# jason-gideon/GPUMounter

Hardware: AMD Instinct MI355X
Metric: p50_gpu_attach_latency_ms (lower is better)
Workload: dtype none

## Files before the change

gpumounter_amd/_native.py:

```python
from __future__ import annotations

import ctypes as C
import os
import subprocess
import threading
from typing import Optional

LIB_DIR = os.path.join(os.path.dirname(os.path.abspath(__file__)), "_lib")
NATIVE_DIR = os.path.join(os.path.dirname(os.path.dirname(os.path.abspath(__file__))), "native")

_lock = threading.Lock()
_libs: dict = {}


class NativeError(RuntimeError):
    pass


def lib_path(name: str) -> str:
    return os.path.join(LIB_DIR, name)


def build(target: str = "all", quiet: bool = True) -> None:
    import fcntl
# ... 71 lines not shown
def mock_smi() -> C.CDLL:
    lib = _load("libamd_smi_mock.so", "host")
    lib.gm_mock_set_procs_file.argtypes = [C.c_char_p]
    lib.gm_mock_set_ecc.argtypes = [C.c_uint32, C.c_uint64, C.c_uint64]
    return lib


class DevRule(C.Structure):
    _fields_ = [("type", C.c_char), ("access", C.c_uint8), ("allow", C.c_uint8),
                ("pad", C.c_uint8), ("major", C.c_int32), ("minor", C.c_int32)]


class DevNode(C.Structure):
    _fields_ = [("path", C.c_char * 112), ("major", C.c_uint32), ("minor", C.c_uint32),
                ("mode", C.c_uint32), ("uid", C.c_int32), ("gid", C.c_int32)]


class BpfTiming(C.Structure):
    _fields_ = [("query_ns", C.c_uint64), ("map_ns", C.c_uint64), ("build_ns", C.c_uint64),
                ("load_ns", C.c_uint64), ("attach_ns", C.c_uint64), ("programs", C.c_uint32),
                ("insns", C.c_uint32)]


HOST_ABI_VERSION = 6
GM_ACC_MKNOD, GM_ACC_READ, GM_ACC_WRITE = 1, 2, 4
GM_DEV_EMULATE, GM_DEV_VIA_SETNS, GM_DEV_REPLACE, GM_DEV_BIND = 1, 2, 4, 8


def host() -> C.CDLL:
    lib = _load("libgm_host.so", "host")
    if not getattr(lib, "_gm_typed", False):
        abi = lib.gm_host_abi_version()
        if abi != HOST_ABI_VERSION:
            raise RuntimeError(f"libgm_host.so ABI {abi} != {HOST_ABI_VERSION} expected: stale "
                               f"build, run `make -C native`")
        lib.gm_cg1_apply.argtypes = [C.c_char_p, C.POINTER(DevRule), C.c_int]
        lib.gm_cg1_format_rule.argtypes = [C.POINTER(DevRule), C.c_char_p, C.c_int]
        lib.gm_bpf_dev_build.argtypes = [C.POINTER(DevRule), C.c_int, C.c_int, C.c_int,
                                         C.POINTER(C.c_uint64), C.c_int]
        lib.gm_bpf_dev_load.argtypes = [C.POINTER(C.c_uint64), C.c_int, C.c_char_p, C.c_char_p,
                                        C.c_int]
        lib.gm_bpf_dev_query.argtypes = [C.c_char_p, C.POINTER(C.c_uint32), C.c_uint32,
                                         C.POINTER(C.c_uint32), C.POINTER(C.c_uint32)]
        lib.gm_bpf_prog_name.argtypes = [C.c_uint32, C.c_char_p, C.c_int]
        lib.gm_bpf_dev_program.argtypes = [C.c_char_p, C.POINTER(C.c_uint64), C.c_uint32,
                                           C.POINTER(C.c_uint32), C.POINTER(C.c_uint32)]
        lib.gm_bpf_dev_program_at.argtypes = [C.c_char_p, C.c_uint32, C.c_int,
# ... 5 lines not shown
                                           C.POINTER(C.c_uint32), C.POINTER(C.c_uint32)]
        lib.gm_bpf_dev_restore.argtypes = [C.c_char_p, C.c_char_p]
        lib.gm_bpf_dev_build_set.argtypes = [C.c_int, C.POINTER(DevRule), C.c_int, C.c_int,
                                             C.c_int, C.POINTER(C.c_uint64), C.c_int]
        lib.gm_bpf_dev_probe_set.argtypes = []
        lib.gm_devnodes_bind_probe.argtypes = []
        lib.gm_bpf_dev_straight_line.argtypes = [C.c_int]
        lib.gm_bpf_dev_straight_line.restype = None
        lib.gm_bpf_dev_set_at.argtypes = [C.c_char_p, C.c_uint32, C.POINTER(C.c_uint32),
                                          C.c_uint32, C.POINTER(C.c_uint32),
                                          C.POINTER(C.c_uint32)]
        lib.gm_bpf_dev_last_timing.argtypes = [C.POINTER(BpfTiming)]
        lib.gm_bpf_dev_last_timing.restype = None
        lib.gm_devnodes_create.argtypes = [C.c_int, C.c_char_p, C.POINTER(DevNode), C.c_int,
                                           C.c_int, C.POINTER(C.c_int)]
        lib.gm_devnodes_remove.argtypes = lib.gm_devnodes_create.argtypes
        lib.gm_devnodes_guard.argtypes = [C.c_char_p]
        lib.gm_devnodes_stage.argtypes = [C.c_char_p, C.c_int]
        lib.gm_devnode_stat.argtypes = [C.c_int, C.c_char_p, C.c_char_p, C.c_int,
                                        C.POINTER(C.c_int), C.POINTER(C.c_uint32),
                                        C.POINTER(C.c_uint32), C.POINTER(C.c_uint32)]
        lib.gm_devnodes_present.argtypes = [C.c_int, C.c_char_p, C.POINTER(DevNode), C.c_int,
                                            C.c_int, C.POINTER(C.c_uint8)]
        lib.gm_proc_dev_users.argtypes = [C.c_uint32, C.c_uint32, C.POINTER(C.c_int32), C.c_int,
                                          C.POINTER(C.c_int)]
        lib.gm_proc_scan_devs.argtypes = [C.POINTER(C.c_int32), C.c_int, C.POINTER(C.c_uint32),
                                          C.c_int, C.POINTER(C.c_uint8), C.POINTER(C.c_int32)]
        lib.gm_proc_filter_dev_users.argtypes = [C.POINTER(C.c_int32), C.c_int, C.c_uint32,
                                                 C.c_uint32, C.POINTER(C.c_int32)]
        lib.gm_proc_read_pids.argtypes = [C.c_char_p, C.POINTER(C.c_int32), C.c_int,
                                          C.POINTER(C.c_int)]
        lib.gm_sd_get_device_allow.argtypes = [C.c_char_p, C.c_char_p, C.c_char_p, C.c_int,
                                               C.c_char_p, C.c_int]
        lib.gm_sd_set_device_allow.argtypes = [C.c_char_p, C.c_char_p, C.POINTER(C.c_char_p),
                                               C.POINTER(C.c_char_p), C.c_int, C.c_int,
                                               C.c_char_p, C.c_int]
        lib.gm_sd_unit_path.argtypes = [C.c_char_p, C.c_char_p, C.c_int]
        lib.gm_roctx_push.argtypes = [C.c_char_p]
        lib.gm_roctx_mark.argtypes = [C.c_char_p]
        lib.gm_roctx_start.argtypes = [C.c_char_p]
        lib.gm_roctx_start.restype = C.c_uint64
        lib.gm_roctx_stop.argtypes = [C.c_uint64]
        lib.gm_roctx_stop.restype = None
        lib.gm_now_ns.restype = C.c_uint64
        lib._gm_typed = True
    return lib
# ... 125 lines not shown
```

gpumounter_amd/node/cgroup.py:

```python
from __future__ import annotations

import ctypes as C
import errno
import functools
import glob
import json
import os
from abc import ABC, abstractmethod
from typing import Dict, FrozenSet, Iterable, List, Optional, Sequence, Set, Tuple

from gpumounter_amd import _native
from gpumounter_amd.models.device import DeviceNode
from gpumounter_amd.models.pod import (QOS_BESTEFFORT, QOS_BURSTABLE, ContainerRef, qos_class,
                                       uid_of)
from gpumounter_amd.node import bpfvm
from gpumounter_amd.utils import log, trace

_log = log.get("node.cgroup")

RUNTIME_SCOPE_PREFIXES = ("cri-containerd-", "docker-", "crio-", "containerd-", "")
FAKE_MARKER = ".gm_fake"
BPF_STATE = "gm.bpf.json"


class CgroupError(RuntimeError):
    pass


def _esc(s: str) -> str:
    return s.replace("-", "_")


class CgroupResolver:
    def __init__(self, root: str = "/sys/fs/cgroup", mode: str = "auto", driver: str = "auto",
                 proc_root: str = "/proc"):
        self.root = root
        self.proc_root = proc_root
        self.mode = self.detect_mode(root) if mode == "auto" else mode
        self.base = os.path.join(root, "devices") if self.mode == "v1" else root
        self.driver = driver
        self._cache: Dict[Tuple[str, str], str] = {}

    @staticmethod
    def detect_mode(root: str) -> str:
        if os.path.isdir(os.path.join(root, "devices")):
            return "v1"
        if os.path.exists(os.path.join(root, "cgroup.controllers")):
            return "v2"
        return "v2"
# ... 60 lines not shown
                with open(os.path.join(self.proc_root, pid, "cgroup")) as fh:
                    lines = fh.read().splitlines()
            except OSError:
                continue
            for line in lines:
                parts = line.split(":", 2)
                if len(parts) != 3 or container_id not in parts[2]:
                    continue
                ctrls = parts[1].split(",") if parts[1] else [""]
                if want_ctrl not in ctrls:
                    continue
                cand = os.path.join(self.base, parts[2].lstrip("/"))
                if os.path.isdir(cand):
                    return cand
        return None

    def forget(self, pod_uid: str) -> None:
        for k in [k for k in self._cache if k[0] == pod_uid]:
            del self._cache[k]

    @staticmethod
    def pids(cgdir: str, recursive: bool = True) -> List[int]:
        lib = _native.host()
        out: List[int] = []
        buf = (C.c_int32 * 4096)()
        n = C.c_int(0)
        stack = [cgdir]
        while stack:
            d = stack.pop()
            path = os.path.join(d, "cgroup.procs")
            rc = lib.gm_proc_read_pids(path.encode(), buf, 4096, C.byref(n))
            if rc < 0 and rc != -errno.ENOENT:
                raise CgroupError(f"read {path}: {os.strerror(-rc)}")
            if rc >= 0:
                out.extend(buf[:min(n.value, 4096)])
            if recursive:
                try:
                    with os.scandir(d) as it:
                        stack.extend(e.path for e in it if e.is_dir(follow_symlinks=False))
                except (FileNotFoundError, NotADirectoryError):
                    pass
        return sorted(set(out))


def rules_for(nodes: Iterable[DeviceNode], allow: bool, access: str = "rw") -> List[_native.DevRule]:
    acc = 0
    if "r" in access:
        acc |= _native.GM_ACC_READ
    if "w" in access:
        acc |= _native.GM_ACC_WRITE
    if "m" in access:
        acc |= _native.GM_ACC_MKNOD
    return [_native.DevRule(b"c", acc, 1 if allow else 0, 0, n.major, n.minor) for n in nodes]


def _rule_array(rules: Sequence[_native.DevRule]):
    arr = (_native.DevRule * max(len(rules), 1))()
    for i, r in enumerate(rules):
        arr[i] = r
    return arr


def format_rule(r: _native.DevRule) -> str:
    buf = C.create_string_buffer(64)
    _native.host().gm_cg1_format_rule(C.byref(r), buf, 64)
# ... 434 lines not shown
```

gpumounter_amd/node/devnodes.py:

```python
from __future__ import annotations

import ctypes as C
import errno
import os
from dataclasses import dataclass
from typing import List, Optional, Sequence, Tuple

from gpumounter_amd import _native
from gpumounter_amd.models.device import DeviceNode
from gpumounter_amd.utils import log


class DevNodeError(RuntimeError):
    def __init__(self, msg: str, results: Sequence[int] = ()):
        super().__init__(msg)
        self.results = list(results)


@dataclass(frozen=True)
class Target:

    pid: int = 0
    root: str = ""


CREATED, PRESENT, SHARED_HOST = 0, 1, 2

_log = log.get("node.devnodes")


class DevNodeWriter:

    def __init__(self, mode: str = "procroot", host_dev: str = "", userns: str = "auto",
                 stage_dir: str = "", proc_root: str = "/proc") -> None:
        self.mode = mode
        self.userns = userns
        self.stage_dir = stage_dir
        self.proc_root = proc_root
        self._staged = False
        self._own_userns = self._userns_id("self")
        self.flags = 0
        if mode == "setns":
            self.flags |= _native.GM_DEV_VIA_SETNS
        if mode == "emulate":
            self.flags |= _native.GM_DEV_EMULATE
        self.host_dev = host_dev
        rc = _native.host().gm_devnodes_guard(host_dev.encode() if host_dev else None)
        if rc < 0:
            _log.warning("host /dev guard off: cannot read %s (%s)", host_dev, os.strerror(-rc))
        self.guarded = max(rc, 0)

    @staticmethod
    def _array(nodes: Sequence[DeviceNode], owner: Tuple[int, int] = (-1, -1)):
        arr = (_native.DevNode * max(len(nodes), 1))()
        for i, n in enumerate(nodes):
            rel = n.path.lstrip("/").encode()
            if len(rel) >= 112:
                raise DevNodeError(f"path too long: {n.path}")
            arr[i].path = rel
            arr[i].major = n.major
            arr[i].minor = n.minor
            arr[i].mode = n.mode
            arr[i].uid, arr[i].gid = owner
        return arr

    def _mntns(self, pid) -> Optional[str]:
        try:
            return os.readlink(f"{self.proc_root}/{pid}/ns/mnt")
        except OSError:
            return None

    def root_pid(self, pids: Sequence[int]) -> int:
        if self.mode == "emulate":
            return pids[0] if pids else 0
        own = self._mntns("self")
        for pid in pids:
            ns = self._mntns(pid)
            if ns is not None and ns != own:
                return pid
        return 0

    def _userns_id(self, pid) -> Optional[Tuple[int, int]]:
        try:
            st = os.stat(f"{self.proc_root}/{pid}/ns/user")
        except OSError:
            return None
        return st.st_dev, st.st_ino

    def _bind(self, t: Target) -> bool:
        if self.userns == "bind":
            return True
        if self.userns != "auto" or self.mode == "emulate" or t.root or t.pid <= 0:
            return False
        theirs = self._userns_id(t.pid)
        return theirs is not None and self._own_userns is not None and theirs != self._own_userns

    def _mapped_root(self, t: Target) -> Tuple[int, int]:
        if t.pid <= 0:
            return -1, -1
        out = []
        for f in ("uid_map", "gid_map"):
            host = -1
            try:
# ... 17 lines not shown
        try:
            os.makedirs(os.path.dirname(self.stage_dir.rstrip("/")) or "/", exist_ok=True)
        except OSError as e:
            raise DevNodeError(f"staging directory {self.stage_dir}: {e.strerror}") from e
        rc = _native.host().gm_devnodes_stage(self.stage_dir.encode(), 1)
        if rc < 0:
            raise DevNodeError(f"staging tmpfs at {self.stage_dir}: {os.strerror(-rc)}")
        self._staged = True

    def _call(self, t: Target):
        if not self._bind(t):
            return self.flags, (-1, -1)
        self._ensure_stage()
        return self.flags | _native.GM_DEV_BIND, self._mapped_root(t)

    def _target_args(self, t: Target) -> Tuple[int, Optional[bytes]]:
        if t.root:
            return 0, t.root.encode()
        if t.pid <= 0:
            raise DevNodeError("container has no process to resolve its root from "
                               "(empty cgroup.procs)")
        return t.pid, None

    def create(self, t: Target, nodes: Sequence[DeviceNode]) -> List[int]:
        if not nodes:
            return []
        pid, root = self._target_args(t)
        flags, owner = self._call(t)
        res = (C.c_int * len(nodes))()
        fails = _native.host().gm_devnodes_create(pid, root, self._array(nodes, owner),
                                                  len(nodes), flags, res)
        results = [int(res[i]) for i in range(len(nodes))]
        if fails:
            bad = [(n.path, os.strerror(-r)) for n, r in zip(nodes, results) if r < 0]
            what = "bind mount" if flags & _native.GM_DEV_BIND else "mknod"
            raise DevNodeError(f"{what} failed: {bad}", results)
        return results

    def remove(self, t: Target, nodes: Sequence[DeviceNode]) -> List[int]:
        if not nodes:
            return []
        pid, root = self._target_args(t)
        flags, _ = self._call(t)
        res = (C.c_int * len(nodes))()
        fails = _native.host().gm_devnodes_remove(pid, root, self._array(nodes), len(nodes),
                                                  flags, res)
        results = [int(res[i]) for i in range(len(nodes))]
        if fails and not flags & _native.GM_DEV_BIND and \
                any(r == -errno.EBUSY for r in results) and self.mode != "emulate":
            busy = [i for i, r in enumerate(results) if r == -errno.EBUSY]
            self._ensure_stage()
            sub = [nodes[i] for i in busy]
            res2 = (C.c_int * len(sub))()
            _native.host().gm_devnodes_remove(pid, root, self._array(sub), len(sub),
                                              flags | _native.GM_DEV_BIND, res2)
            for k, i in enumerate(busy):
                results[i] = int(res2[k])
            fails = sum(1 for r in results if r < 0)
        if fails:
            if all(r in (-errno.ESRCH, -errno.ENOENT) for r in results if r < 0):
# ... 37 lines not shown
```

gpumounter_amd/node/hotmount.py:

```python
from __future__ import annotations

import os
from dataclasses import dataclass, field
from typing import Dict, List, Optional, Sequence

from gpumounter_amd.hw.inventory import Inventory
from gpumounter_amd.models.device import AmdGpu, DeviceNode, kfd_node
from gpumounter_amd.models.pod import ContainerRef, running_containers
from gpumounter_amd.node.cgroup import CgroupError, CgroupResolver, DeviceRuleBackend
from gpumounter_amd.node.devnodes import CREATED, DevNodeError, DevNodeWriter, Target
from gpumounter_amd.node.journal import InjectionJournal
from gpumounter_amd.utils import log, trace

_log = log.get("node.hotmount")


class MountError(RuntimeError):
    pass


@dataclass
class ContainerTarget:
    ref: ContainerRef
    cgdir: str
    target: Target
    pids: List[int] = field(default_factory=list)


@dataclass
class AuditIssue:
    container: str
    kind: str
    path: str
    major: int
    minor: int


class HotMount:
    def __init__(self, cfg, inv: Inventory, resolver: CgroupResolver, backend: DeviceRuleBackend,
                 writer: DevNodeWriter, faults=None,
                 journal: Optional[InjectionJournal] = None) -> None:
        from gpumounter_amd.utils.faults import NONE

        self.cfg = cfg
        self.inv = inv
        self.resolver = resolver
        self.backend = backend
        self.writer = writer
        self.faults = faults if faults is not None else NONE
        self.journal = journal if journal is not None else InjectionJournal()
        self.expected: Dict[str, object] = {}

    def _apply(self, cgdir: str, grant, revoke, desired) -> None:
        try:
            self.backend.apply(cgdir, grant, revoke, desired)
        finally:
            fp = getattr(self.backend, "fingerprint", None)
            self.expected[cgdir] = fp(cgdir) if fp is not None else None

    def kfd(self) -> DeviceNode:
        return kfd_node(self.inv.kfd_major)

    def gpu_nodes(self, gpus: Sequence[AmdGpu]) -> List[DeviceNode]:
        out: List[DeviceNode] = []
        for g in sorted(gpus, key=lambda g: g.index):
            out.extend(g.device_nodes(self.cfg.drm_major, self.cfg.inject_card_nodes,
                                      self.cfg.device_file_mode))
        return out

    def managed_nodes(self, hot: Sequence[AmdGpu], base: Sequence[AmdGpu]) -> List[DeviceNode]:
        base_keys = {(n.major, n.minor) for n in self.gpu_nodes(base)}
        nodes = [n for n in self.gpu_nodes(hot) if (n.major, n.minor) not in base_keys]
        if hot and not base:
            nodes.insert(0, self.kfd())
        return nodes

    def targets(self, pod: dict, container: str = "",
                include_privileged: bool = False) -> List[ContainerTarget]:
        refs = [r for r in running_containers(pod, container) if r.running]
        if not refs:
            raise MountError(f"pod {pod['metadata'].get('name')} has no running container"
                             + (f" named {container}" if container else ""))
        out = []
        for r in refs:
            if r.privileged and not include_privileged:
                continue
            cgdir = self.resolver.container_dir(pod, r)
            pids = self.resolver.pids(cgdir)
            if self.cfg.container_root_prefix:
                t = Target(root=os.path.join(self.cfg.container_root_prefix, r.id))
            else:
                t = Target(pid=self.writer.root_pid(pids))
            out.append(ContainerTarget(r, cgdir, t, pids))
        return out

    def _owner(self, pod: dict, t: ContainerTarget) -> dict:
        md = pod.get("metadata", {})
# ... 2 lines not shown

    def resolve(self, pod: dict, container: str = "",
                include_privileged: bool = False) -> List[ContainerTarget]:
        try:
            return self.targets(pod, container, include_privileged)
        except (CgroupError, OSError) as e:
            raise MountError(f"cannot resolve the pod's containers: {e}") from e

    def attach(self, pod: dict, new: Sequence[AmdGpu], have: Sequence[AmdGpu],
               base: Sequence[AmdGpu] = (), container: str = "") -> List[ContainerTarget]:
        before = self.managed_nodes(have, base)
        after = self.managed_nodes(list(have) + list(new), base)
        before_keys = {(n.major, n.minor) for n in before}
        grant = [n for n in after if (n.major, n.minor) not in before_keys]
        with trace.span("resolve"):
            targets = self.resolve(pod, container)
        done: List[tuple] = []
        j = self.journal
        try:
            for t in targets:
                cid = t.ref.id
                known = j.nodes_of(cid)
                with trace.span("devnodes_probe", nodes=len(after)):
                    states = self.writer.present_states(t.target, after)
                theirs = {(n.major, n.minor) for n, st in zip(after, states)
                          if st and (n.major, n.minor) not in known}
                j.intend(cid, [((n.major, n.minor), n.path) for n in grant],
                         [((n.major, n.minor), n.path) for n in after
                          if (n.major, n.minor) not in theirs], **self._owner(pod, t))
                done.append((t, grant, []))
                with trace.span("cgroup_rule", backend=self.backend.name, rules=len(grant)):
                    self.faults.check("cgroup_rule")
                    self._apply(t.cgdir, grant, [], after)
                self.faults.check("cgroup_rule", "after")
                with trace.span("devnodes", nodes=len(after)):
                    self.faults.check("devnodes")
                    res = self.writer.create(t.target, after)
                done[-1] = (t, grant, [n for n, r in zip(after, res) if r == CREATED])
                j.settle(cid, [(n.major, n.minor) for n, r in zip(after, res)
                               if r != CREATED and (n.major, n.minor) not in known
                               and (n.major, n.minor) not in theirs])
                self.faults.check("devnodes", "after")
        except Exception as e:
            self._rollback_attach(done, before)
            for t in targets[len(done):]:
                self._forget_new(t.ref.id, grant, after, before)
            raise MountError(f"attach failed, rolled back: {e}") from e
        return targets

    def _forget_new(self, cid: str, granted, after, before) -> None:
        keep = {(n.major, n.minor) for n in before}
        self.journal.forget(cid, [(n.major, n.minor) for n in granted],
                            [(n.major, n.minor) for n in after if (n.major, n.minor) not in keep])

    def _rollback_attach(self, done, before: List[DeviceNode]) -> None:
        before_keys = {(n.major, n.minor) for n in before}
        for t, granted, created in reversed(done):
            try:
                self.writer.remove(t.target, created)
            except Exception as e:
                _log.error("rollback unlink in %s failed: %s", t.ref.name, e)
            else:
                self.journal.forget(t.ref.id, (), [(n.major, n.minor) for n in created
                                                   if (n.major, n.minor) not in before_keys])
            try:
                try:
                    have = self.backend.installed(t.cgdir)
                    revoke = [n for n in granted if (n.major, n.minor) in have]
                except Exception:
                    revoke = list(granted)
                if revoke:
# ... 105 lines not shown
        if rules:
            self._apply(t.cgdir, [], rules, [])
            self.journal.forget(container_id, [(n.major, n.minor) for n in rules])
        if nodes:
            self.writer.remove(t.target, nodes)
            self.journal.forget(container_id, (), [(n.major, n.minor) for n in nodes])
        return out

    def verify(self, pod: dict, hot: Sequence[AmdGpu], base: Sequence[AmdGpu] = (),
               container: str = "",
               targets: Optional[List[ContainerTarget]] = None) -> List[AuditIssue]:
        want = self.managed_nodes(hot, base)
        issues: List[AuditIssue] = []
        try:
            return self._verify(want, targets if targets is not None
                                else self.targets(pod, container), issues)
        except (CgroupError, DevNodeError, OSError) as e:
            raise MountError(f"read-back failed: {e}") from e

    def _verify(self, want: List[DeviceNode], targets: List[ContainerTarget],
                issues: List[AuditIssue]) -> List[AuditIssue]:
        for t in targets:
            allowed = self.backend.allowed(t.cgdir)
            present = self.writer.present_many(t.target, want)
            for n, ok in zip(want, present):
                if (n.major, n.minor) not in allowed:
                    issues.append(AuditIssue(t.ref.name, "missing_rule", n.path, n.major, n.minor))
                if not ok:
                    issues.append(AuditIssue(t.ref.name, "missing_node", n.path, n.major, n.minor))
        return issues

    def audit(self, pod: dict, hot: Sequence[AmdGpu], base: Sequence[AmdGpu] = (),
              container: str = "") -> List[AuditIssue]:
        want = self.managed_nodes(hot, base)
        want_keys = {(n.major, n.minor) for n in want}
        issues: List[AuditIssue] = []
        base_keys = {(n.major, n.minor) for n in self.gpu_nodes(base)}
        for t in self.targets(pod, container):
            allowed = self.backend.allowed(t.cgdir)
            for n, ok in zip(want, self.writer.present_many(t.target, want)):
                if (n.major, n.minor) not in allowed:
                    issues.append(AuditIssue(t.ref.name, "missing_rule", n.path, n.major, n.minor))
                if not ok:
                    issues.append(AuditIssue(t.ref.name, "missing_node", n.path, n.major, n.minor))
            ent = self.journal.get(t.ref.id)
            if ent is None:
                continue
# ... 21 lines not shown
```

gpumounter_amd/node/journal.py:

```python
from __future__ import annotations

import json
import os
import threading
import time
from dataclasses import dataclass, field
from typing import Dict, Iterable, List, Optional, Tuple

from gpumounter_amd.utils import log

_log = log.get("node.journal")

Key = Tuple[int, int]


@dataclass
class Entry:
    container_id: str
    namespace: str = ""
    pod: str = ""
    pod_uid: str = ""
    container: str = ""
    cgdir: str = ""
    rules: Dict[Key, str] = field(default_factory=dict)
    nodes: Dict[Key, str] = field(default_factory=dict)
    updated: float = 0.0

    def empty(self) -> bool:
        return not self.rules and not self.nodes

    def to_json(self) -> dict:
        return {"container_id": self.container_id, "namespace": self.namespace, "pod": self.pod,
                "pod_uid": self.pod_uid, "container": self.container, "cgdir": self.cgdir,
                "rules": sorted([ma, mi, p] for (ma, mi), p in self.rules.items()),
                "nodes": sorted([ma, mi, p] for (ma, mi), p in self.nodes.items()),
                "updated": self.updated}

    @classmethod
    def from_json(cls, d: dict) -> "Entry":
        return cls(d["container_id"], d.get("namespace", ""), d.get("pod", ""),
                   d.get("pod_uid", ""), d.get("container", ""), d.get("cgdir", ""),
                   {(int(a), int(b)): p for a, b, p in d.get("rules", [])},
                   {(int(a), int(b)): p for a, b, p in d.get("nodes", [])},
                   float(d.get("updated", 0.0)))


def _safe_id(cid: str) -> bool:
    return bool(cid) and all(c.isalnum() or c in "-_." for c in cid) and cid[0] != "."


class InjectionJournal:
    def __init__(self, state_dir: str = "") -> None:
        self.dir = state_dir
        self._entries: Dict[str, Entry] = {}
        self._mu = threading.Lock()
        self.writes = 0
        if state_dir:
            os.makedirs(state_dir, mode=0o700, exist_ok=True)
            self._load()

    def _path(self, cid: str) -> str:
        return os.path.join(self.dir, cid + ".json")

    def _load(self) -> None:
        for fn in os.listdir(self.dir):
            if not fn.endswith(".json"):
                continue
            try:
                with open(os.path.join(self.dir, fn), encoding="utf-8") as fh:
                    e = Entry.from_json(json.load(fh))
# ... 108 lines not shown
```

gpumounter_amd/worker/service.py:

```python
from __future__ import annotations

import asyncio
import contextlib
import json
import secrets
import time
import weakref
from dataclasses import dataclass, field
from typing import Dict, List, Optional, Sequence, Tuple

import grpc

from gpumounter_amd.api import gpu_mount as api
from gpumounter_amd.cluster.correction import Correction, ReserveGate, placement_worse
from gpumounter_amd.cluster.informer import PodInformer
from gpumounter_amd.cluster.kube import ApiError, KubeClient, NotFound
from gpumounter_amd.cluster.placeholder import (InsufficientGPU, Placeholder, PlaceholderManager,
                                                ReserveError)
from gpumounter_amd.cluster.quota import GpuQuota, QuotaExceeded
from gpumounter_amd.hw import topology
from gpumounter_amd.hw.inventory import Inventory
from gpumounter_amd.models import pod as podu
from gpumounter_amd.models.device import AmdGpu, normalize_device_id
from gpumounter_amd.models.types import (ANN_ATTACH_ID, ANN_IDEMPOTENCY, ANN_MOUNT_MODE,
# ... 434 lines not shown
                _log.info("quota refused %d GPU(s) for %s/%s: %s", n, req.namespace,
                          req.pod_name, e)
                self.notify.event(pod, "GPUAttachFailed", str(e), warning=True)
                raise RpcError(grpc.StatusCode.RESOURCE_EXHAUSTED, f"{ERR_QUOTA}: {e}") from e
            except InsufficientGPU as e:
                _log.info("insufficient GPUs on %s: %s", self.cfg.node_name, e)
                self.notify.event(pod, "GPUAttachFailed",
                                  f"{n} GPU(s) requested, node {self.cfg.node_name} cannot "
                                  f"provide them: {e}", warning=True)
                return api.AddGPUResponse(add_gpu_result=api.ADD_INSUFFICIENT, message=str(e))
            except (ReserveError, asyncio.TimeoutError, InjectedFault, LedgerError) as e:
                self._follow_up(pod)
                raise RpcError(grpc.StatusCode.INTERNAL, f"{ERR_INTERNAL}: {e}") from e
            keys = self.inv.by_key()
            new = [keys[normalize_device_id(d)] for d in res.device_ids]
            owner = {}
            for ph in res.placeholders:
                for d in ph.device_ids:
                    owner[keys[normalize_device_id(d)].index] = ph.name
            want = res.preferred or preferred
            if want and sorted(normalize_device_id(d) for d in res.device_ids) != \
                    sorted(normalize_device_id(d) for d in want):
                self.metrics.placement_mismatch.inc()
            try:
                pod = self._current(pod)
                with trace.span("mount", gpus=len(new)):
                    targets = self.hm.attach(pod, new, st.hot, st.own, req.container)
                if self.cfg.attach_verify:
                    with trace.span("verify"):
                        self.faults.check("verify")
                        issues = self.hm.verify(pod, list(st.hot) + new, st.own,
                                                req.container, targets)
                    if issues:
                        self.metrics.verify_failures.inc()
                        raise MountError("attach did not take effect: " + ", ".join(
                            f"{i.container}:{i.kind}:{i.path}" for i in issues[:4]))
            except (MountError, InjectedFault) as e:
                _log.error("mount failed on %s/%s: %s", req.namespace, req.pod_name, e)
                await self._release_or_follow_up(pod, res.placeholders, "a failed mount")
                if await self._rollback(pod, "attach"):
                    return api.AddGPUResponse(add_gpu_result=api.ADD_POD_NOT_FOUND,
                                              message=f"pod went away during the attach: {e}")
                raise RpcError(grpc.StatusCode.INTERNAL, f"{ERR_INTERNAL}: {e}") from e
            if self._owner_gone(pod):
                _log.warning("pod %s/%s was deleted during the attach; releasing its GPUs",
                             req.namespace, req.pod_name)
                await self._release_or_follow_up(pod, res.placeholders, "an attach into a "
                                                                         "deleted pod")
                return api.AddGPUResponse(add_gpu_result=api.ADD_POD_NOT_FOUND,
                                          message="pod went away during the attach")
            msg = "Add GPU Success"
            if lease_exp:
                lease_exp = await self._lease_booked(pod, res.placeholders, lease_exp,
                                                     req.lease_s)
                msg += time.strftime(" (lease until %Y-%m-%dT%H:%M:%SZ)", time.gmtime(lease_exp))
            log.kv(_log, 20, "attached", pod=f"{req.namespace}/{req.pod_name}",
                   gpus=[g.bdf for g in new], by=req.requested_by, lease_s=req.lease_s)
            self.notify.attached(pod, new, list(st.hot) + new,
                                 "entire" if req.is_entire_mount else "single",
# ... 414 lines not shown
```

native/include/gm_host.h:

```cpp
#pragma once
#include <stdint.h>

#ifdef __cplusplus
extern "C" {
#endif

#define GM_HOST_ABI_VERSION 6

#define GM_ACC_MKNOD 1
#define GM_ACC_READ 2
#define GM_ACC_WRITE 4

typedef struct gm_dev_rule {
  char type;
  uint8_t access;
  uint8_t allow;
  uint8_t pad;
  int32_t major;
  int32_t minor;
} gm_dev_rule_t;

int gm_cg1_apply(const char* cgdir, const gm_dev_rule_t* rules, int n);
int gm_cg1_format_rule(const gm_dev_rule_t* rule, char* out, int cap);

int gm_bpf_dev_build(const gm_dev_rule_t* rules, int n, int default_allow, int chain_map_fd,
                     uint64_t* out, int cap);
int gm_bpf_dev_build_set(int set_map_fd, const gm_dev_rule_t* base, int nbase, int default_allow,
                         int chain_map_fd, uint64_t* out, int cap);
int gm_bpf_dev_load(const uint64_t* insns, int n, const char* name, char* log, int logcap);
int gm_bpf_dev_query(const char* cgroup_path, uint32_t* ids, uint32_t cap, uint32_t* n,
// ... 24 lines not shown
  uint32_t minor;
  uint32_t mode;
  int32_t uid;
  int32_t gid;
} gm_dev_node_t;

#define GM_DEV_EMULATE 1
#define GM_DEV_VIA_SETNS 2
#define GM_DEV_REPLACE 4
#define GM_DEV_BIND 8

int gm_devnodes_guard(const char* host_dev);
int gm_devnodes_stage(const char* dir, int mount_tmpfs);
int gm_devnodes_bind_probe(void);
int gm_devnodes_create(int pid, const char* root, const gm_dev_node_t* nodes, int n, int flags,
                       int* results);
int gm_devnodes_remove(int pid, const char* root, const gm_dev_node_t* nodes, int n, int flags,
                       int* results);
int gm_devnode_stat(int pid, const char* root, const char* path, int flags, int* kind,
                    uint32_t* major, uint32_t* minor, uint32_t* mode);
int gm_devnodes_present(int pid, const char* root, const gm_dev_node_t* nodes, int n, int flags,
                        uint8_t* present);

int gm_proc_dev_users(uint32_t major, uint32_t minor, int32_t* pids, int cap, int* n);
int gm_proc_scan_devs(const int32_t* pids, int n, const uint32_t* majmin, int ndev,
                      uint8_t* hits, int32_t* unreadable);
int gm_proc_filter_dev_users(const int32_t* pids, int n, uint32_t major, uint32_t minor,
                             int32_t* out);
int gm_proc_read_pids(const char* path, int32_t* pids, int cap, int* n);

int gm_sd_get_device_allow(const char* bus_path, const char* unit, char* out, int cap, char* err,
                           int errcap);
int gm_sd_set_device_allow(const char* bus_path, const char* unit, const char* const* paths,
                           const char* const* perms, int n, int reset, char* err, int errcap);
int gm_sd_unit_path(const char* unit, char* out, int cap);

int gm_roctx_available(void);
void gm_roctx_push(const char* name);
void gm_roctx_pop(void);
void gm_roctx_mark(const char* name);
uint64_t gm_roctx_start(const char* name);
void gm_roctx_stop(uint64_t id);
uint64_t gm_now_ns(void);

int gm_host_abi_version(void);

#ifdef __cplusplus
}
#endif
```

native/src/gm_host.cpp:

```cpp
#include "gm_host.h"

#include <dirent.h>
#include <dlfcn.h>
#include <errno.h>
#include <fcntl.h>
#include <linux/bpf.h>
#include <sched.h>
#include <signal.h>
#include <stdio.h>
#include <stdlib.h>
#include <string.h>
#include <sys/mount.h>
#include <sys/stat.h>
#include <sys/syscall.h>
#include <sys/sysmacros.h>
#include <time.h>
#include <unistd.h>

#include <atomic>
#include <map>
#include <mutex>
#include <string>
#include <thread>
#include <vector>

namespace {

constexpr const char* kProgName = "gm_devallow";

struct Fd {
  int fd = -1;
  Fd() = default;
  explicit Fd(int f) : fd(f) {}
  Fd(const Fd&) = delete;
  Fd& operator=(const Fd&) = delete;
  Fd(Fd&& o) noexcept : fd(o.fd) { o.fd = -1; }
  Fd& operator=(Fd&& o) noexcept {
    if (this != &o) {
      reset();
      fd = o.fd;
      o.fd = -1;
// ... 797 lines not shown
  std::string leaf;
  int e = w.parent(n.path, false, &pfd, &leaf);
  if (e == -ENOENT) return 1;
  if (e != 0) return e;
  if (guarded_dir(pfd)) return kSharedHost;
  int kind;
  uint32_t maj, min, mode;
  e = stat_leaf(pfd, leaf, &kind, &maj, &min, &mode);
  if (e < 0) return e;
  if (kind == 0) return 1;
  int mounted = is_mount_leaf(pfd, leaf);
  if (mounted < 0) return mounted;
  if (!mounted) {
    if (kind == 3 && is_placeholder(pfd, leaf)) {
      if (unlinkat(pfd, leaf.c_str(), 0) < 0) return -errno;
      return 0;
    }
    return remove_one(w, n);
  }
  if (!(kind == 1 && maj == n.major && min == n.minor)) return -EEXIST;
  if ((e = unmount_leaf(pfd, leaf)) < 0) return e;
  if (is_placeholder(pfd, leaf) && unlinkat(pfd, leaf.c_str(), 0) < 0) return -errno;
  return 0;
}

struct Roctx {
  std::once_flag once;
  int (*push)(const char*) = nullptr;
  int (*pop)() = nullptr;
  void (*mark)(const char*) = nullptr;
  uint64_t (*start)(const char*) = nullptr;
  void (*stop)(uint64_t) = nullptr;
};
Roctx g_roctx;

void roctx_init() {
  std::call_once(g_roctx.once, []() {
    const char* env = getenv("GM_ROCTX");
    if (env && strcmp(env, "0") == 0) return;
    const char* libs[] = {"librocprofiler-sdk-roctx.so.1", "librocprofiler-sdk-roctx.so",
                          "/opt/rocm/lib/librocprofiler-sdk-roctx.so.1"};
    void* dl = nullptr;
    for (const char* l : libs) {
      dl = dlopen(l, RTLD_NOW | RTLD_GLOBAL);
      if (dl) break;
    }
// ... 497 lines not shown
  }
  int fd = open(dir, O_PATH | O_DIRECTORY | O_NOFOLLOW | O_CLOEXEC);
  if (fd < 0) return -errno;
  g_stage_fd = fd;
  return 0;
}

int gm_devnodes_create(int pid, const char* root, const gm_dev_node_t* nodes, int n, int flags,
                       int* results) {
  int failures = 0;
  std::vector<Fd> trees;
  if (flags & GM_DEV_BIND) {
    for (int i = 0; i < n; ++i) {
      int t = staged_tree(nodes[i]);
      if (t < 0) {
        for (int j = 0; j < n; ++j) results[j] = t;
        return n;
      }
      trees.emplace_back(t);
    }
  }
  int e = with_root(pid, root, flags, [&](int rootfd) {
    Walker w(rootfd);
    for (int i = 0; i < n; ++i) {
      results[i] = (flags & GM_DEV_BIND) ? create_bound(w, nodes[i], trees[i].fd, flags)
                                         : create_one(w, nodes[i], flags);
      if (results[i] < 0) ++failures;
    }
    return 0;
  });
  if (e < 0) {
    for (int i = 0; i < n; ++i) results[i] = e;
    return n;
  }
  return failures;
}

int gm_devnodes_remove(int pid, const char* root, const gm_dev_node_t* nodes, int n, int flags,
                       int* results) {
  int failures = 0;
  int e = with_root(pid, root, flags, [&](int rootfd) {
    Walker w(rootfd);
    for (int i = 0; i < n; ++i) {
      results[i] = (flags & GM_DEV_BIND) ? remove_bound(w, nodes[i]) : remove_one(w, nodes[i]);
      if (results[i] < 0) ++failures;
    }
    return 0;
  });
  if (e < 0) {
    for (int i = 0; i < n; ++i) results[i] = e;
    return n;
// ... 2 lines not shown
}

int gm_devnode_stat(int pid, const char* root, const char* path, int flags, int* kind,
                    uint32_t* maj, uint32_t* min, uint32_t* mode) {
  return with_root(pid, root, flags, [&](int rootfd) {
    Fd parent;
    std::string leaf;
    int e = walk_parent(rootfd, path, false, &parent, &leaf);
    if (e == -ENOENT) {
      *kind = 0;
      *maj = *min = *mode = 0;
      return 0;
    }
    if (e < 0) return e;
    return stat_leaf(parent.fd, leaf, kind, maj, min, mode);
  });
}

int gm_devnodes_present(int pid, const char* root, const gm_dev_node_t* nodes, int n, int flags,
                        uint8_t* present) {
  int count = 0;
  int e = with_root(pid, root, flags, [&](int rootfd) {
    Walker wk(rootfd);
    for (int i = 0; i < n; ++i) {
      present[i] = 0;
      int pfd;
      std::string leaf;
      int w = wk.parent(nodes[i].path, false, &pfd, &leaf);
      if (w == -ENOENT) {
        std::string dir(nodes[i].path);
        const size_t cut = dir.rfind('/');
        dir = cut == std::string::npos ? std::string() : dir.substr(0, cut);
        Fd d2;
        std::string l2;
        if (!dir.empty() && walk_parent(rootfd, dir.c_str(), false, &d2, &l2) == 0 &&
            guarded_dir(d2.fd)) {
          present[i] = kSharedHost;
          ++count;
        }
        continue;
      }
      if (w < 0) continue;
      if (guarded_dir(pfd)) {
        present[i] = kSharedHost;
        ++count;
        continue;
      }
      int kind = 0;
      uint32_t ma = 0, mi = 0, mode = 0;
      if (stat_leaf(pfd, leaf, &kind, &ma, &mi, &mode) < 0) continue;
      if ((kind == 1 || kind == 2) && ma == nodes[i].major && mi == nodes[i].minor &&
          (!(flags & GM_DEV_BIND) || is_mount_leaf(pfd, leaf) == 1)) {
        present[i] = 1;
        ++count;
      }
    }
    return 0;
  });
  return e < 0 ? e : count;
}

namespace {
bool pid_uses_dev(long pid, dev_t want) {
  char p[64];
  snprintf(p, sizeof(p), "/proc/%ld/fd", pid);
  int dfd = open(p, O_RDONLY | O_DIRECTORY | O_CLOEXEC);
  if (dfd < 0) return false;
  DIR* fds = fdopendir(dfd);
  if (!fds) {
    close(dfd);
    return false;
  }
  struct dirent* fe;
  bool hit = false;
  while (!hit && (fe = readdir(fds)) != nullptr) {
    if (fe->d_name[0] == '.') continue;
    struct stat st;
    if (fstatat(dirfd(fds), fe->d_name, &st, 0) == 0 && S_ISCHR(st.st_mode) && st.st_rdev == want)
      hit = true;
  }
  closedir(fds);
  return hit;
}
// ... 54 lines not shown
    const bool hit = pid_uses_dev(pid, want);
    if (hit) {
      if (*n < cap) pids[*n] = (int32_t)pid;
      ++*n;
    }
  }
  closedir(proc);
  return 0;
}

int gm_proc_read_pids(const char* path, int32_t* pids, int cap, int* n) {
  *n = 0;
  FILE* f = fopen(path, "re");
  if (!f) return -errno;
  long v;
  while (fscanf(f, "%ld", &v) == 1) {
    if (*n < cap) pids[*n] = (int32_t)v;
    ++*n;
  }
  fclose(f);
  return 0;
}

int gm_roctx_available(void) {
  roctx_init();
  return g_roctx.push != nullptr;
}
void gm_roctx_push(const char* name) {
  roctx_init();
  if (g_roctx.push) g_roctx.push(name);
}
void gm_roctx_pop(void) {
  roctx_init();
  if (g_roctx.pop) g_roctx.pop();
}
uint64_t gm_roctx_start(const char* name) {
  roctx_init();
  return g_roctx.start ? g_roctx.start(name) : 0;
}
void gm_roctx_stop(uint64_t id) {
  roctx_init();
  if (g_roctx.stop && id) g_roctx.stop(id);
}
void gm_roctx_mark(const char* name) {
  roctx_init();
  if (g_roctx.mark) g_roctx.mark(name);
// ... 9 lines not shown
```

Baseline: 1.101.

## Reuse device-node sessions and move cgroup pid and mntns scans native

New measurement: 1.110. No clear change (+0.8%).

```diff
diff --git a/gpumounter_amd/_native.py b/gpumounter_amd/_native.py
--- a/gpumounter_amd/_native.py
+++ b/gpumounter_amd/_native.py
@@ -117,7 +117,7 @@
                 ("insns", C.c_uint32)]
 
 
-HOST_ABI_VERSION = 6
+HOST_ABI_VERSION = 7
 GM_ACC_MKNOD, GM_ACC_READ, GM_ACC_WRITE = 1, 2, 4
 GM_DEV_EMULATE, GM_DEV_VIA_SETNS, GM_DEV_REPLACE, GM_DEV_BIND = 1, 2, 4, 8
 
@@ -169,6 +169,17 @@
                                         C.POINTER(C.c_uint32), C.POINTER(C.c_uint32)]
         lib.gm_devnodes_present.argtypes = [C.c_int, C.c_char_p, C.POINTER(DevNode), C.c_int,
                                             C.c_int, C.POINTER(C.c_uint8)]
+        lib.gm_devsession_open.argtypes = [C.c_int, C.c_char_p, C.POINTER(DevNode), C.c_int,
+                                           C.c_int, C.POINTER(C.c_void_p)]
+        lib.gm_devsession_probe.argtypes = [C.c_void_p, C.POINTER(C.c_uint8)]
+        lib.gm_devsession_create.argtypes = [C.c_void_p, C.POINTER(C.c_int)]
+        lib.gm_devsession_present.argtypes = [C.c_void_p, C.POINTER(C.c_uint8)]
+        lib.gm_devsession_close.argtypes = [C.c_void_p]
+        lib.gm_devsession_close.restype = None
+        lib.gm_devsession_live.argtypes = []
+        lib.gm_cgroup_pids.argtypes = [C.c_char_p, C.c_int, C.POINTER(C.c_int32), C.c_int,
+                                       C.POINTER(C.c_int)]
+        lib.gm_proc_root_pid.argtypes = [C.c_char_p, C.POINTER(C.c_int32), C.c_int]
         lib.gm_proc_dev_users.argtypes = [C.c_uint32, C.c_uint32, C.POINTER(C.c_int32), C.c_int,
                                           C.POINTER(C.c_int)]
         lib.gm_proc_scan_devs.argtypes = [C.POINTER(C.c_int32), C.c_int, C.POINTER(C.c_uint32),
diff --git a/gpumounter_amd/node/cgroup.py b/gpumounter_amd/node/cgroup.py
--- a/gpumounter_amd/node/cgroup.py
+++ b/gpumounter_amd/node/cgroup.py
@@ -6,6 +6,7 @@
 import glob
 import json
 import os
+import threading
 from abc import ABC, abstractmethod
 from typing import Dict, FrozenSet, Iterable, List, Optional, Sequence, Set, Tuple
 
@@ -25,6 +26,9 @@
 
 class CgroupError(RuntimeError):
     pass
+
+
+_pid_buf = threading.local()
 
 
 def _esc(s: str) -> str:
@@ -131,25 +135,18 @@
     @staticmethod
     def pids(cgdir: str, recursive: bool = True) -> List[int]:
         lib = _native.host()
-        out: List[int] = []
-        buf = (C.c_int32 * 4096)()
         n = C.c_int(0)
-        stack = [cgdir]
-        while stack:
-            d = stack.pop()
-            path = os.path.join(d, "cgroup.procs")
-            rc = lib.gm_proc_read_pids(path.encode(), buf, 4096, C.byref(n))
-            if rc < 0 and rc != -errno.ENOENT:
-                raise CgroupError(f"read {path}: {os.strerror(-rc)}")
-            if rc >= 0:
-                out.extend(buf[:min(n.value, 4096)])
-            if recursive:
-                try:
-                    with os.scandir(d) as it:
-                        stack.extend(e.path for e in it if e.is_dir(follow_symlinks=False))
-                except (FileNotFoundError, NotADirectoryError):
-                    pass
-        return sorted(set(out))
+        path = cgdir.encode()
+        while True:
+            buf = getattr(_pid_buf, "buf", None)
+            if buf is None:
+                buf = _pid_buf.buf = (C.c_int32 * 256)()
+            rc = lib.gm_cgroup_pids(path, 1 if recursive else 0, buf, len(buf), C.byref(n))
+            if rc < 0:
+                raise CgroupError(f"read cgroup.procs under {cgdir}: {os.strerror(-rc)}")
+            if n.value <= len(buf):
+                return buf[:n.value]
+            _pid_buf.buf = (C.c_int32 * (2 * n.value))()
 
 
 def rules_for(nodes: Iterable[DeviceNode], allow: bool, access: str = "rw") -> List[_native.DevRule]:
diff --git a/gpumounter_amd/node/devnodes.py b/gpumounter_amd/node/devnodes.py
--- a/gpumounter_amd/node/devnodes.py
+++ b/gpumounter_amd/node/devnodes.py
@@ -27,6 +27,47 @@
 CREATED, PRESENT, SHARED_HOST = 0, 1, 2
 
 _log = log.get("node.devnodes")
+
+
+class DevNodeSession:
+
+    def __init__(self, handle, nodes: List[DeviceNode], flags: int) -> None:
+        self._h = handle
+        self._lib = _native.host()
+        self.nodes = nodes
+        self.flags = flags
+
+    def _handle(self):
+        if self._h is None:
+            raise DevNodeError("device-node session used after close")
+        return self._h
+
+    def probe(self) -> List[int]:
+        out = (C.c_uint8 * len(self.nodes))()
+        rc = self._lib.gm_devsession_probe(self._handle(), out)
+        if rc < 0:
+            raise DevNodeError(f"read-back of {len(self.nodes)} nodes: {os.strerror(-rc)}")
+        return list(out)
+
+    def create(self) -> List[int]:
+        res = (C.c_int * len(self.nodes))()
+        fails = self._lib.gm_devsession_create(self._handle(), res)
+        return DevNodeWriter._create_results(self.nodes, res, fails, self.flags)
+
+    def present(self) -> List[bool]:
+        out = (C.c_uint8 * len(self.nodes))()
+        rc = self._lib.gm_devsession_present(self._handle(), out)
+        if rc < 0:
+            raise DevNodeError(f"read-back of {len(self.nodes)} nodes: {os.strerror(-rc)}")
+        return [bool(s) for s in out]
+
+    def close(self) -> None:
+        h, self._h = self._h, None
+        if h is not None:
+            self._lib.gm_devsession_close(h)
+
+    def __del__(self) -> None:
+        self.close()
 
 
 class DevNodeWriter:
@@ -73,12 +114,10 @@
     def root_pid(self, pids: Sequence[int]) -> int:
         if self.mode == "emulate":
             return pids[0] if pids else 0
-        own = self._mntns("self")
-        for pid in pids:
-            ns = self._mntns(pid)
-            if ns is not None and ns != own:
-                return pid
-        return 0
+        if not pids:
+            return 0
+        arr = (C.c_int32 * len(pids))(*pids)
+        return int(_native.host().gm_proc_root_pid(self.proc_root.encode(), arr, len(pids)))
 
     def _userns_id(self, pid) -> Optional[Tuple[int, int]]:
         try:
@@ -142,20 +181,41 @@
                                "(empty cgroup.procs)")
         return t.pid, None
 
-    def create(self, t: Target, nodes: Sequence[DeviceNode]) -> List[int]:
-        if not nodes:
-            return []
-        pid, root = self._target_args(t)
-        flags, owner = self._call(t)
-        res = (C.c_int * len(nodes))()
-        fails = _native.host().gm_devnodes_create(pid, root, self._array(nodes, owner),
-                                                  len(nodes), flags, res)
+    @staticmethod
+    def _create_results(nodes: Sequence[DeviceNode], res, fails: int, flags: int) -> List[int]:
         results = [int(res[i]) for i in range(len(nodes))]
         if fails:
             bad = [(n.path, os.strerror(-r)) for n, r in zip(nodes, results) if r < 0]
             what = "bind mount" if flags & _native.GM_DEV_BIND else "mknod"
             raise DevNodeError(f"{what} failed: {bad}", results)
         return results
+
+    def create(self, t: Target, nodes: Sequence[DeviceNode]) -> List[int]:
+        if not nodes:
+            return []
+        pid, root = self._target_args(t)
+        flags, owner = self._call(t)
+        res = (C.c_int * len(nodes))()
+        fails = _native.host().gm_devnodes_create(pid, root, self._array(nodes, owner),
+                                                  len(nodes), flags, res)
+        return self._create_results(nodes, res, fails, flags)
+
+    def open_session(self, t: Target, nodes: Sequence[DeviceNode]) -> Optional["DevNodeSession"]:
+        if not nodes:
+            return None
+        for name in ("present_states", "create", "present_many"):
+            if getattr(getattr(self, name), "__func__", None) is not getattr(DevNodeWriter, name):
+                return None
+        pid, root = self._target_args(t)
+        flags, owner = self._call(t)
+        handle = C.c_void_p()
+        rc = _native.host().gm_devsession_open(pid, root, self._array(nodes, owner), len(nodes),
+                                               flags, C.byref(handle))
+        if rc == -errno.ENOTSUP:
+            return None
+        if rc < 0:
+            raise DevNodeError(f"read-back of {len(nodes)} nodes: {os.strerror(-rc)}")
+        return DevNodeSession(handle, list(nodes), flags)
 
     def remove(self, t: Target, nodes: Sequence[DeviceNode]) -> List[int]:
         if not nodes:
diff --git a/gpumounter_amd/node/hotmount.py b/gpumounter_amd/node/hotmount.py
--- a/gpumounter_amd/node/hotmount.py
+++ b/gpumounter_amd/node/hotmount.py
@@ -25,6 +25,7 @@
     cgdir: str
     target: Target
     pids: List[int] = field(default_factory=list)
+    session = None
 
 
 @dataclass
@@ -50,6 +51,7 @@
         self.faults = faults if faults is not None else NONE
         self.journal = journal if journal is not None else InjectionJournal()
         self.expected: Dict[str, object] = {}
+        self._managed: Dict[tuple, tuple] = {}
 
     def _apply(self, cgdir: str, grant, revoke, desired) -> None:
         try:
@@ -69,10 +71,21 @@
         return out
 
     def managed_nodes(self, hot: Sequence[AmdGpu], base: Sequence[AmdGpu]) -> List[DeviceNode]:
+        cfg = self.cfg
+        key = (tuple((g.index, g.render_minor, g.card_minor) for g in hot),
+               tuple((g.index, g.render_minor, g.card_minor) for g in base),
+               cfg.drm_major, cfg.inject_card_nodes, cfg.device_file_mode,
+               getattr(self.inv, "kfd_major", None))
+        hit = self._managed.get(key)
+        if hit is not None:
+            return list(hit)
         base_keys = {(n.major, n.minor) for n in self.gpu_nodes(base)}
         nodes = [n for n in self.gpu_nodes(hot) if (n.major, n.minor) not in base_keys]
         if hot and not base:
             nodes.insert(0, self.kfd())
+        if len(self._managed) >= 256:
+            self._managed.clear()
+        self._managed[key] = tuple(nodes)
         return nodes
 
     def targets(self, pod: dict, container: str = "",
@@ -121,7 +134,12 @@
                 cid = t.ref.id
                 known = j.nodes_of(cid)
                 with trace.span("devnodes_probe", nodes=len(after)):
-                    states = self.writer.present_states(t.target, after)
+                    opener = getattr(self.writer, "open_session", None)
+                    t.session = opener(t.target, after) if opener is not None else None
+                    if t.session is not None:
+                        states = t.session.probe()
+                    else:
+                        states = self.writer.present_states(t.target, after)
                 theirs = {(n.major, n.minor) for n, st in zip(after, states)
                           if st and (n.major, n.minor) not in known}
                 j.intend(cid, [((n.major, n.minor), n.path) for n in grant],
@@ -134,18 +152,34 @@
                 self.faults.check("cgroup_rule", "after")
                 with trace.span("devnodes", nodes=len(after)):
                     self.faults.check("devnodes")
-                    res = self.writer.create(t.target, after)
+                    try:
+                        if t.session is not None:
+                            res = t.session.create()
+                        else:
+                            res = self.writer.create(t.target, after)
+                    except DevNodeError as e:
+                        done[-1] = (t, grant, [n for n, r in zip(after, e.results)
+                                               if r == CREATED])
+                        raise
                 done[-1] = (t, grant, [n for n, r in zip(after, res) if r == CREATED])
                 j.settle(cid, [(n.major, n.minor) for n, r in zip(after, res)
                                if r != CREATED and (n.major, n.minor) not in known
                                and (n.major, n.minor) not in theirs])
                 self.faults.check("devnodes", "after")
         except Exception as e:
+            self.release(targets)
             self._rollback_attach(done, before)
             for t in targets[len(done):]:
                 self._forget_new(t.ref.id, grant, after, before)
             raise MountError(f"attach failed, rolled back: {e}") from e
         return targets
+
+    @staticmethod
+    def release(targets: Optional[Sequence[ContainerTarget]]) -> None:
+        for t in targets or ():
+            s, t.session = getattr(t, "session", None), None
+            if s is not None:
+                s.close()
 
     def _forget_new(self, cid: str, granted, after, before) -> None:
         keep = {(n.major, n.minor) for n in before}
@@ -297,7 +331,11 @@
                 issues: List[AuditIssue]) -> List[AuditIssue]:
         for t in targets:
             allowed = self.backend.allowed(t.cgdir)
-            present = self.writer.present_many(t.target, want)
+            s = getattr(t, "session", None)
+            if s is not None and s.nodes == want:
+                present = s.present()
+            else:
+                present = self.writer.present_many(t.target, want)
             for n, ok in zip(want, present):
                 if (n.major, n.minor) not in allowed:
                     issues.append(AuditIssue(t.ref.name, "missing_rule", n.path, n.major, n.minor))
diff --git a/gpumounter_amd/node/journal.py b/gpumounter_amd/node/journal.py
--- a/gpumounter_amd/node/journal.py
+++ b/gpumounter_amd/node/journal.py
@@ -2,6 +2,7 @@
 
 import json
 import os
+import re
 import threading
 import time
 from dataclasses import dataclass, field
@@ -45,7 +46,12 @@
                    float(d.get("updated", 0.0)))
 
 
+_SAFE_ID_FAST = re.compile(r"[A-Za-z0-9_-][A-Za-z0-9_.-]*\Z")
+
+
 def _safe_id(cid: str) -> bool:
+    if _SAFE_ID_FAST.match(cid):
+        return True
     return bool(cid) and all(c.isalnum() or c in "-_." for c in cid) and cid[0] != "."
 
 
diff --git a/gpumounter_amd/worker/service.py b/gpumounter_amd/worker/service.py
--- a/gpumounter_amd/worker/service.py
+++ b/gpumounter_amd/worker/service.py
@@ -480,19 +480,23 @@
             if want and sorted(normalize_device_id(d) for d in res.device_ids) != \
                     sorted(normalize_device_id(d) for d in want):
                 self.metrics.placement_mismatch.inc()
+            targets = None
             try:
                 pod = self._current(pod)
-                with trace.span("mount", gpus=len(new)):
-                    targets = self.hm.attach(pod, new, st.hot, st.own, req.container)
-                if self.cfg.attach_verify:
-                    with trace.span("verify"):
-                        self.faults.check("verify")
-                        issues = self.hm.verify(pod, list(st.hot) + new, st.own,
-                                                req.container, targets)
-                    if issues:
-                        self.metrics.verify_failures.inc()
-                        raise MountError("attach did not take effect: " + ", ".join(
-                            f"{i.container}:{i.kind}:{i.path}" for i in issues[:4]))
+                try:
+                    with trace.span("mount", gpus=len(new)):
+                        targets = self.hm.attach(pod, new, st.hot, st.own, req.container)
+                    if self.cfg.attach_verify:
+                        with trace.span("verify"):
+                            self.faults.check("verify")
+                            issues = self.hm.verify(pod, list(st.hot) + new, st.own,
+                                                    req.container, targets)
+                        if issues:
+                            self.metrics.verify_failures.inc()
+                            raise MountError("attach did not take effect: " + ", ".join(
+                                f"{i.container}:{i.kind}:{i.path}" for i in issues[:4]))
+                finally:
+                    self.hm.release(targets)
             except (MountError, InjectedFault) as e:
                 _log.error("mount failed on %s/%s: %s", req.namespace, req.pod_name, e)
                 await self._release_or_follow_up(pod, res.placeholders, "a failed mount")
diff --git a/native/include/gm_host.h b/native/include/gm_host.h
--- a/native/include/gm_host.h
+++ b/native/include/gm_host.h
@@ -5,7 +5,7 @@
 extern "C" {
 #endif
 
-#define GM_HOST_ABI_VERSION 6
+#define GM_HOST_ABI_VERSION 7
 
 #define GM_ACC_MKNOD 1
 #define GM_ACC_READ 2
@@ -76,12 +76,23 @@
 int gm_devnodes_present(int pid, const char* root, const gm_dev_node_t* nodes, int n, int flags,
                         uint8_t* present);
 
+typedef struct gm_devsession gm_devsession_t;
+int gm_devsession_open(int pid, const char* root, const gm_dev_node_t* nodes, int n, int flags,
+                       gm_devsession_t** out);
+int gm_devsession_probe(gm_devsession_t* s, uint8_t* states);
+int gm_devsession_create(gm_devsession_t* s, int* results);
+int gm_devsession_present(gm_devsession_t* s, uint8_t* present);
+void gm_devsession_close(gm_devsession_t* s);
+int gm_devsession_live(void);
+
 int gm_proc_dev_users(uint32_t major, uint32_t minor, int32_t* pids, int cap, int* n);
 int gm_proc_scan_devs(const int32_t* pids, int n, const uint32_t* majmin, int ndev,
                       uint8_t* hits, int32_t* unreadable);
 int gm_proc_filter_dev_users(const int32_t* pids, int n, uint32_t major, uint32_t minor,
                              int32_t* out);
 int gm_proc_read_pids(const char* path, int32_t* pids, int cap, int* n);
+int gm_cgroup_pids(const char* cgdir, int recursive, int32_t* pids, int cap, int* n);
+int gm_proc_root_pid(const char* proc_root, const int32_t* pids, int n);
 
 int gm_sd_get_device_allow(const char* bus_path, const char* unit, char* out, int cap, char* err,
                            int errcap);
diff --git a/native/src/gm_host.cpp b/native/src/gm_host.cpp
--- a/native/src/gm_host.cpp
+++ b/native/src/gm_host.cpp
@@ -17,6 +17,7 @@
 #include <time.h>
 #include <unistd.h>
 
+#include <algorithm>
 #include <atomic>
 #include <map>
 #include <mutex>
@@ -860,6 +861,129 @@
   if ((e = unmount_leaf(pfd, leaf)) < 0) return e;
   if (is_placeholder(pfd, leaf) && unlinkat(pfd, leaf.c_str(), 0) < 0) return -errno;
   return 0;
+}
+
+std::string dir_of(const char* path) {
+  std::string p(path);
+  const size_t cut = p.rfind('/');
+  return cut == std::string::npos ? std::string() : p.substr(0, cut);
+}
+
+int create_all(Walker& w, const gm_dev_node_t* nodes, int n, int flags,
+               const std::vector<Fd>* trees, bool rewalk, int* results) {
+  int failures = 0;
+  for (int i = 0; i < n; ++i) {
+    int r = (flags & GM_DEV_BIND) ? create_bound(w, nodes[i], (*trees)[i].fd, flags)
+                                  : create_one(w, nodes[i], flags);
+    if (r == -ENOENT && rewalk && !(flags & GM_DEV_BIND)) {
+      w.dirs.clear();
+      r = create_one(w, nodes[i], flags);
+    }
+    results[i] = r;
+    if (r < 0) ++failures;
+  }
+  return failures;
+}
+
+int present_all(Walker& wk, const gm_dev_node_t* nodes, int n, int flags, uint8_t* present) {
+  int count = 0;
+  for (int i = 0; i < n; ++i) {
+    present[i] = 0;
+    int pfd;
+    std::string leaf;
+    int w = wk.parent(nodes[i].path, false, &pfd, &leaf);
+    if (w == -ENOENT) {
+      const std::string dir = dir_of(nodes[i].path);
+      Fd d2;
+      std::string l2;
+      if (!dir.empty() && walk_parent(wk.rootfd, dir.c_str(), false, &d2, &l2) == 0 &&
+          guarded_dir(d2.fd)) {
+        present[i] = kSharedHost;
+        ++count;
+      }
+      continue;
+    }
+    if (w < 0) continue;
+    if (guarded_dir(pfd)) {
+      present[i] = kSharedHost;
+      ++count;
+      continue;
+    }
+    int kind = 0;
+    uint32_t ma = 0, mi = 0, mode = 0;
+    if (stat_leaf(pfd, leaf, &kind, &ma, &mi, &mode) < 0) continue;
+    if ((kind == 1 || kind == 2) && ma == nodes[i].major && mi == nodes[i].minor &&
+        (!(flags & GM_DEV_BIND) || is_mount_leaf(pfd, leaf) == 1)) {
+      present[i] = 1;
+      ++count;
+    }
+  }
+  return count;
+}
+
+std::atomic<int> g_sessions_live{0};
+
+int read_procs_at(int dirfd, std::vector<int32_t>* out) {
+  Fd f(openat(dirfd, "cgroup.procs", O_RDONLY | O_CLOEXEC));
+  if (!f.ok()) return errno == ENOENT ? 0 : -errno;
+  char buf[4096];
+  long v = 0;
+  bool in_num = false;
+  for (;;) {
+    ssize_t r = read(f.fd, buf, sizeof(buf));
+    if (r < 0) {
+      if (errno == EINTR) continue;
+      return -errno;
+    }
+    if (r == 0) break;
+    for (ssize_t i = 0; i < r; ++i) {
+      const char c = buf[i];
+      if (c >= '0' && c <= '9') {
+        v = v * 10 + (c - '0');
+        if (v > INT32_MAX) return -ERANGE;
+        in_num = true;
+      } else {
+        if (in_num) out->push_back((int32_t)v);
+        v = 0;
+        in_num = false;
+        if (c != '\n' && c != ' ' && c != '\t' && c != '\r') return 0;
+      }
+    }
+  }
+  if (in_num) out->push_back((int32_t)v);
+  return 0;
+}
+
+constexpr int kCgroupMaxDepth = 64;
+
+int walk_cgroup(Fd dir, bool recursive, int depth, std::vector<int32_t>* out) {
+  int e = read_procs_at(dir.fd, out);
+  if (e < 0 || !recursive) return e;
+  if (depth >= kCgroupMaxDepth) return -ELOOP;
+  DIR* d = fdopendir(dir.fd);
+  if (!d) return -errno;
+  dir.fd = -1;
+  int rc = 0;
+  for (;;) {
+    errno = 0;
+    struct dirent* de = readdir(d);
+    if (!de) {
+      if (errno) rc = -errno;
+      break;
+    }
+    const char* nm = de->d_name;
+    if (nm[0] == '.' && (nm[1] == 0 || (nm[1] == '.' && nm[2] == 0))) continue;
+    if (de->d_type != DT_DIR && de->d_type != DT_UNKNOWN) continue;
+    Fd sub(openat(dirfd(d), nm, O_RDONLY | O_DIRECTORY | O_NOFOLLOW | O_CLOEXEC));
+    if (!sub.ok()) {
+      if (errno == ENOENT || errno == ENOTDIR || errno == ELOOP) continue;
+      rc = -errno;
+      break;
+    }
+    if ((rc = walk_cgroup(std::move(sub), true, depth + 1, out)) < 0) break;
+  }
+  closedir(d);
+  return rc;
 }
 
 struct Roctx {
@@ -1403,11 +1527,7 @@
   }
   int e = with_root(pid, root, flags, [&](int rootfd) {
     Walker w(rootfd);
-    for (int i = 0; i < n; ++i) {
-      results[i] = (flags & GM_DEV_BIND) ? create_bound(w, nodes[i], trees[i].fd, flags)
-                                         : create_one(w, nodes[i], flags);
-      if (results[i] < 0) ++failures;
-    }
+    failures = create_all(w, nodes, n, flags, &trees, false, results);
     return 0;
   });
   if (e < 0) {
@@ -1456,43 +1576,57 @@
   int count = 0;
   int e = with_root(pid, root, flags, [&](int rootfd) {
     Walker wk(rootfd);
-    for (int i = 0; i < n; ++i) {
-      present[i] = 0;
-      int pfd;
-      std::string leaf;
-      int w = wk.parent(nodes[i].path, false, &pfd, &leaf);
-      if (w == -ENOENT) {
-        std::string dir(nodes[i].path);
-        const size_t cut = dir.rfind('/');
-        dir = cut == std::string::npos ? std::string() : dir.substr(0, cut);
-        Fd d2;
-        std::string l2;
-        if (!dir.empty() && walk_parent(rootfd, dir.c_str(), false, &d2, &l2) == 0 &&
-            guarded_dir(d2.fd)) {
-          present[i] = kSharedHost;
-          ++count;
-        }
-        continue;
-      }
-      if (w < 0) continue;
-      if (guarded_dir(pfd)) {
-        present[i] = kSharedHost;
-        ++count;
-        continue;
-      }
-      int kind = 0;
-      uint32_t ma = 0, mi = 0, mode = 0;
-      if (stat_leaf(pfd, leaf, &kind, &ma, &mi, &mode) < 0) continue;
-      if ((kind == 1 || kind == 2) && ma == nodes[i].major && mi == nodes[i].minor &&
-          (!(flags & GM_DEV_BIND) || is_mount_leaf(pfd, leaf) == 1)) {
-        present[i] = 1;
-        ++count;
-      }
-    }
+    count = present_all(wk, nodes, n, flags, present);
     return 0;
   });
   return e < 0 ? e : count;
 }
+
+struct gm_devsession {
+  Fd root;
+  std::vector<gm_dev_node_t> nodes;
+  int flags;
+  Walker w;
+  gm_devsession(int rootfd, const gm_dev_node_t* ns, int n, int fl)
+      : root(rootfd), nodes(ns, ns + n), flags(fl), w(rootfd) {}
+};
+
+int gm_devsession_open(int pid, const char* root, const gm_dev_node_t* nodes, int n, int flags,
+                       gm_devsession_t** out) {
+  if (!out || n < 0 || (n > 0 && !nodes)) return -EINVAL;
+  *out = nullptr;
+  const bool explicit_root = root && *root;
+  if ((flags & GM_DEV_BIND) || ((flags & GM_DEV_VIA_SETNS) && !explicit_root)) return -ENOTSUP;
+  int rfd = open_root(pid, root);
+  if (rfd < 0) return rfd;
+  *out = new gm_devsession(rfd, nodes, n, flags);
+  g_sessions_live.fetch_add(1, std::memory_order_relaxed);
+  return 0;
+}
+
+int gm_devsession_probe(gm_devsession_t* s, uint8_t* states) {
+  if (!s) return -EINVAL;
+  return present_all(s->w, s->nodes.data(), (int)s->nodes.size(), s->flags, states);
+}
+
+int gm_devsession_create(gm_devsession_t* s, int* results) {
+  if (!s) return -EINVAL;
+  return create_all(s->w, s->nodes.data(), (int)s->nodes.size(), s->flags, nullptr, true, results);
+}
+
+int gm_devsession_present(gm_devsession_t* s, uint8_t* present) {
+  if (!s) return -EINVAL;
+  Walker fresh(s->root.fd);
+  return present_all(fresh, s->nodes.data(), (int)s->nodes.size(), s->flags, present);
+}
+
+void gm_devsession_close(gm_devsession_t* s) {
+  if (!s) return;
+  delete s;
+  g_sessions_live.fetch_sub(1, std::memory_order_relaxed);
+}
+
+int gm_devsession_live(void) { return g_sessions_live.load(std::memory_order_relaxed); }
 
 namespace {
 bool pid_uses_dev(long pid, dev_t want) {
@@ -1593,6 +1727,32 @@
   return 0;
 }
 
+int gm_cgroup_pids(const char* cgdir, int recursive, int32_t* pids, int cap, int* n) {
+  *n = 0;
+  Fd top(open(cgdir, O_RDONLY | O_DIRECTORY | O_CLOEXEC));
+  if (!top.ok()) return errno == ENOENT ? 0 : -errno;
+  std::vector<int32_t> all;
+  int e = walk_cgroup(std::move(top), recursive != 0, 0, &all);
+  if (e < 0) return e;
+  std::sort(all.begin(), all.end());
+  all.erase(std::unique(all.begin(), all.end()), all.end());
+  *n = (int)all.size();
+  for (int i = 0; i < *n && i < cap; ++i) pids[i] = all[(size_t)i];
+  return 0;
+}
+
+int gm_proc_root_pid(const char* proc_root, const int32_t* pids, int n) {
+  const std::string base(proc_root && *proc_root ? proc_root : "/proc");
+  char own[128], ns[128];
+  ssize_t ol = readlink((base + "/self/ns/mnt").c_str(), own, sizeof(own));
+  for (int i = 0; i < n; ++i) {
+    ssize_t l = readlink((base + "/" + std::to_string(pids[i]) + "/ns/mnt").c_str(), ns, sizeof(ns));
+    if (l < 0) continue;
+    if (l != ol || memcmp(ns, own, (size_t)l) != 0) return pids[i];
+  }
+  return 0;
+}
+
 int gm_roctx_available(void) {
   roctx_init();
   return g_roctx.push != nullptr;
```
